# KELVIN-ASU/Lightweight-Multi-Modal-Scene-Understanding-via-Knowledge-Distillation

Measured on AMD Instinct MI355X. Metric: PandaSet 2-class KD training frames/sec, higher is better.
Workload: dtype f32; 1 GPU; KD step: concat-fusion teacher fwd (eval) -> weighted-fusion student fwd/bwd (train BN), CE + T^2*KL(T=4) + feature-MSE, fused AdamW; random-init weights; teacher_fusion=concat, student_fusion=weighted, image=3x256x256, points_per_frame=80000, bev_grid=64x64, num_classes=2, per_gpu_batch=256, global_batch=256, parallelism=dp1

## Files before the change

include/kd_hip.h:

```cpp
#ifndef KD_HIP_H
#define KD_HIP_H
#include <stddef.h>
#include <stdint.h>

#ifdef __cplusplus
extern "C" {
#endif

#define KD_ACT_NONE 0
#define KD_ACT_RELU 1
#define KD_ACT_RELU6 2

int kd_version(void);
const char* kd_arch(void);
const char* kd_last_error_string(void);

int kd_set_gemm_split(int on);
int64_t kd_pwconv_stat_rows(int64_t M);
int64_t kd_pwconv_stat_rows_for(int64_t M, int K, int N, int pro, int epi, int with_addend);
int kd_set_gemm_stream(int mode);
int kd_pwconv_gemm(const float* A, int64_t lda, const float* A2, int64_t lda2, int pro, int pro_act,
                   const float* p0, const float* p1, const float* p2, const float* p3, const float* p4,
                   const float* W, const float* bias, float* C, int64_t ldc, const float* addend,
                   int64_t ldadd, int epi, const float* X, int64_t ldx, const float* esc, const float* esh,
                   const float* emean, const float* einv, int epi_act, float* partial, int64_t partial_rows, int64_t M,
                   int K, int N, const int* m_dev, void* stream);
size_t kd_pwconv_wgrad_ws_bytes(int64_t M, int N, int K);
int kd_set_wgrad_rs(int mode);
int kd_pwconv_wgrad(const float* D, int64_t ldd, const float* X, int64_t ldx, int d_mode, int d_act,
                    const float* al, const float* be, const float* ga, const float* msc, const float* msh,
                    const float* A, int64_t lda, int a_mode, int a_act, const float* asc, const float* ash,
                    float* dW, int64_t M, int N, int K, void* ws, size_t ws_bytes, void* stream);
int kd_transpose(const float* in, float* out, int R, int C, void* stream);
int kd_transpose_batch(const int64_t* table, int n, int nblocks, void* stream);
int kd_copy_segments(const float* s0, float* d0, int64_t n0, const float* s1, float* d1, int64_t n1, const float* s2, float* d2,
                     int64_t n2, const float* s3, float* d3, int64_t n3, void* stream);

int64_t kd_stem_stat_rows(int64_t npix_out);
int kd_stem_conv_fwd(const float* x_nchw, const float* w, float* y_nhwc, float* partial, int B, int Cin, int H,
                     int W, int Cout, void* stream);
int kd_stem_conv_fwd_infer(const float* x_nchw, const float* w, const float* sc, const float* sh, int act, float* y_nhwc,
                           int B, int Cin, int H, int W, int Cout, void* stream);
int kd_stem_im2col(const float* x_nchw, float* col, int B, int Cin, int H, int W, int Kp, void* stream);

int64_t kd_dwconv_stat_rows(int64_t npix_out, int C);
int kd_dwconv3x3_fwd(const float* x, const float* sc, const float* sh, int act, const float* w, float* y,
                     float* partial, int B, int H, int W, int C, int stride, void* stream);
int64_t kd_dwconv_bwd_stat_rows(int64_t npix_in, int C);
int kd_set_dw_bwd_mode(int mode);
size_t kd_dwconv_bwd_ws_bytes(int64_t npix_out, int C);
int kd_dwconv3x3_bwd(const float* D, const float* Y, const float* al, const float* be, const float* ga,
                     const float* dsc, const float* dsh, int d_act, const float* x, const float* sc,
                     const float* sh, int act, const float* mean, const float* invstd, const float* w, float* gx,
                     float* partial, float* dw, int B, int H, int W, int C, int stride, void* ws, size_t ws_bytes,
                     void* stream);
int kd_dwconv3x3_bwd_add_supported(int C, int W, int stride);
int kd_dwconv3x3_bwd_add(const float* D, const float* Y, const float* al, const float* be, const float* ga,
                         const float* dsc, const float* dsh, int d_act, const float* x, const float* sc,
                         const float* sh, int act, const float* mean, const float* invstd, const float* w,
                         const float* addend, float* gx, float* partial, float* dw, int B, int H, int W, int C, int stride,
                         void* ws, size_t ws_bytes, void* stream);

int kd_bn_finalize_train(float* partial, int rows, int C, int pstride, int64_t count, const float* gamma,
                         const float* beta, float eps, float momentum, float* running_mean, float* running_var,
                         int64_t* num_batches_tracked, float* mean, float* invstd, float* scale, float* shift,
                         void* stream);
int kd_bn_eval_coeffs(const float* gamma, const float* beta, const float* running_mean, const float* running_var,
                      float eps, int C, float* mean, float* invstd, float* scale, float* shift, void* stream);
int64_t kd_rowwise_stat_rows(int64_t M, int C);
int kd_bn_act_apply(const float* x, int64_t ldx, const float* sc, const float* sh, int act, const float* res,
                    int64_t ldr, float* out, int64_t ldo, int64_t M, int C, void* stream);
int kd_bn_act_apply_res(const float* x, int64_t ldx, const float* sc, const float* sh, int act, const float* res, int64_t ldr,
                        const float* rsc, const float* rsh, int ract, float* out, int64_t ldo, int64_t M, int C, void* stream);
int kd_bn_bwd_reduce(const float* D, int64_t ldd, const float* X, int64_t ldx, const float* sc, const float* sh,
                     int act, const float* mean, const float* invstd, float* partial, int64_t M, int C,
                     void* stream);
int kd_bn_bwd_finalize(float* partial, int rows, int C, int pstride, int64_t count, const float* gamma, const float* mean,
                       const float* invstd, int training, float* dgamma, float* dbeta, float* al, float* be,
                       float* ga, float* dbias, void* stream);

int kd_lidar_l0_fwd(const float* pts, const float* w, const float* b, float* y, float* partial, int64_t P, int C,
                    const int* p_dev, void* stream);
int kd_lidar_l1_fwd(const float* pts, const float* w0, const float* b0, const float* sc0, const float* sh0, int act0,
                    const float* W1, const float* bias1, float* C, int64_t ldc, int epi, float* partial,
                    int64_t partial_rows, int64_t M, int K, int N, const int* m_dev, void* stream);
// ... 224 lines not shown
```

lightweight-multi-modal-scene-understanding-via-knowledge-distillation_amd/csrc/kd_wgrad_rs.hip:

```cpp
#include "kd_gemm_args.h"

#include <atomic>

int kd_gemm_split_mode();

namespace {

constexpr int RS_THREADS = 512;

__host__ __device__ constexpr int rs_pad(int blk) { return (blk & 1) ? 64 : 32; }
__host__ __device__ constexpr int rs_pitch(int blk) { return 32 * blk + rs_pad(blk); }
__host__ __device__ constexpr int rs_rpp(int cg, int rows) {
  int r = 256 / cg;
  int p = 1;
  while (p * 2 <= r && p * 2 <= rows) p *= 2;
  return p;
}

struct RsGeom {
  int WN, WK;
  int ncs, split_n;
  int nrs;
  int rows_per_slice;
};

template <int TNW, int TKW, int WNc, int WKc, int CHK, int DMODE, int AMODE>
__global__ __launch_bounds__(RS_THREADS, 1) void pw_wgrad_rs_kernel(WgradArgs g, RsGeom q) {
  constexpr int NBLK = TNW * WNc, KBLK = TKW * WKc;
  constexpr int CH = 16 * CHK;
  constexpr int PD = rs_pitch(NBLK), PA = rs_pitch(KBLK);
  constexpr int PLD = CH * PD, PLA = CH * PA;
  constexpr int BUF = 3 * (PLD + PLA);
  constexpr int CGD = 8 * NBLK, CGA = 8 * KBLK;
  constexpr int RPD = rs_rpp(CGD, CH), RPA = rs_rpp(CGA, CH);
  constexpr int ND = CH / RPD, NA = CH / RPA;
  constexpr int NDT = DMODE == 2 ? 2 : 1;
  extern __shared__ __attribute__((aligned(16))) unsigned char smem_raw[];
  unsigned short* lds = reinterpret_cast<unsigned short*>(smem_raw);
  const int tid = threadIdx.x, lane = tid & 63, wave = tid >> 6;
  int cs, rsl;
  {
    const int grp = 8 * q.ncs, g0 = (int)blockIdx.x / grp, r = (int)blockIdx.x % grp;
    if ((g0 + 1) * 8 <= q.nrs) { rsl = g0 * 8 + (r & 7); cs = r >> 3; }
    else { const int rem = q.nrs - g0 * 8; rsl = g0 * 8 + r % rem; cs = r / rem; }
  }
  const int n0 = q.split_n ? cs * 32 * NBLK : 0, k0 = q.split_n ? 0 : cs * 32 * KBLK;
  const int64_t mbeg = (int64_t)rsl * q.rows_per_slice;
  int64_t mend = mbeg + q.rows_per_slice;
  if (mend > g.M) mend = g.M;
  const int nchunk = mbeg < mend ? (int)((mend - mbeg + CH - 1) / CH) : 0;
  const int nstep = (nchunk + 1) & ~1;

  if (wave < 4) {
    constexpr int ACTD = CGD * RPD, ACTA = CGA * RPA;
    static_assert(ACTD >= 128 && ACTA >= 128 && ACTD <= 256 && ACTA <= 256, "lane map");
    const int td = tid < ACTD ? tid : tid - (256 - ACTD), ta = tid < ACTA ? tid : tid - (256 - ACTA);
    const int dcg = td % CGD, drp = td / CGD;
    const int acg = ta % CGA, arp = ta / CGA;
    const int gn = n0 + 4 * dcg, gk = k0 + 4 * acg;
    float4 cd[DMODE == 2 ? 5 : 1], ca[AMODE == 1 ? 2 : 1];
    if (DMODE == 2) {
      cd[0] = kd_ld4(g.al + gn); cd[1] = kd_ld4(g.be + gn); cd[2] = kd_ld4(g.ga + gn);
      cd[3] = kd_ld4(g.msc + gn); cd[4] = kd_ld4(g.msh + gn);
    }
    if (AMODE == 1) { ca[0] = kd_ld4(g.asc + gk); ca[1] = kd_ld4(g.ash + gk); }
    const float* Dp = g.D + n0;
    const float* Xp = DMODE == 2 ? g.X + n0 : nullptr;
    const float* Ap = g.A + k0;
    const int ldd_ = (int)g.ldd, ldx_ = (int)g.ldx, lda_ = (int)g.lda;
    float4 rd[2][NDT][ND], ra[2][NA];
    auto issue = [&](int c, float4 (&sd)[NDT][ND], float4 (&sa)[NA]) __attribute__((always_inline)) {
      const int cc = c < nchunk ? c : (nchunk > 0 ? nchunk - 1 : 0);
      const int64_t m0 = mbeg + (int64_t)cc * CH;
      const int lastrow = (int)(mend - 1 - m0);
      const float* db = Dp + m0 * g.ldd;
      const float* xb = DMODE == 2 ? Xp + m0 * g.ldx : nullptr;
      const float* ab = Ap + m0 * g.lda;
#pragma unroll
      for (int i = 0; i < ND; ++i) {
        const int r = drp + RPD * i, rr = r < lastrow ? r : lastrow;
        sd[0][i] = kd_ld4(db + (unsigned)(rr * ldd_ + 4 * dcg));
        if (DMODE == 2) sd[1][i] = kd_ld4(xb + (unsigned)(rr * ldx_ + 4 * dcg));
      }
#pragma unroll
      for (int i = 0; i < NA; ++i) {
        const int r = arp + RPA * i, rr = r < lastrow ? r : lastrow;
        sa[i] = kd_ld4(ab + (unsigned)(rr * lda_ + 4 * acg));
      }
    };
    auto split_store = [&](float4 v, unsigned short* d, int plane) __attribute__((always_inline)) {
      uint2 hi, mid, lo;
      kd_split3(v, hi, mid, lo);
      *reinterpret_cast<uint2*>(d) = hi;
      *reinterpret_cast<uint2*>(d + plane) = mid;
      *reinterpret_cast<uint2*>(d + 2 * plane) = lo;
    };
    auto convert = [&](int c, const float4 (&sd)[NDT][ND], const float4 (&sa)[NA], int bufi) __attribute__((always_inline)) {
      unsigned short* bd = lds + bufi * BUF;
      unsigned short* ba = bd + 3 * PLD;
      const int64_t m0 = mbeg + (int64_t)c * CH;
      {
#pragma unroll
        for (int i = 0; i < ND; ++i) {
          const int row = drp + RPD * i;
// ... 90 lines not shown
        }
    }
  }
}

std::atomic<int> g_rs_on{1};
int rs_mode() { return g_rs_on.load(std::memory_order_relaxed); }

struct RsPlan { int tnw, tkw, wn, wk, chk, ncs, split_n; };

bool rs_plan(int N, int K, RsPlan& p, bool any = false) {
  if (N % 32 || K % 32) return false;
  int nb = N / 32, kb = K / 32, ncs = 1, split_n = 0;
  if (nb == 24) { nb = 8; ncs = 3; split_n = 1; }
  else if (kb == 24 && nb == 4) { kb = 12; ncs = 2; }
  else if (kb == 24) { kb = 6; ncs = 4; }
  else if (kb == 12 && nb == 4) { }
  else if (kb == 12 && nb <= 4) { kb = 6; ncs = 2; }
  else if (nb == 8 && kb == 8) { nb = 4; ncs = 2; split_n = 1; }
  struct E { int nb, kb, tnw, tkw, wn, wk, chk; };
  static const E tab[] = {
      {6, 1, 3, 1, 2, 1, 2},
      {12, 2, 3, 2, 4, 1, 1},
      {8, 4, 2, 4, 4, 1, 1},
      {2, 6, 1, 3, 2, 2, 2},
      {4, 12, 1, 12, 4, 1, 1},
      {4, 4, 2, 2, 2, 2, 2},
      {4, 2, 2, 1, 2, 2, 2},
      {2, 4, 1, 2, 2, 2, 2},
      {4, 8, 2, 4, 2, 2, 1},
      {2, 8, 1, 4, 2, 2, 2},
  };
  const bool all = any || rs_mode() == 2;
  for (const E& e : tab)
    if (e.nb == nb && e.kb == kb) {
      const bool wins = (nb == 4 && kb == 12) || (nb == 6 && kb == 1) || (nb == 12 && kb == 2) || (nb == 8 && kb == 4) || (nb == 2 && kb == 6 && ncs == 2) ||
                        (nb == 4 && kb == 8);
      if (!wins && !all) return false;
      p = {e.tnw, e.tkw, e.wn, e.wk, e.chk, ncs, split_n};
      return true;
    }
  return false;
}

template <int TNW, int TKW, int WN, int WK, int CHK>
int rs_launch_shape(const WgradArgs& g, const RsGeom& q, hipStream_t st) {
  constexpr int NBLK = TNW * WN, KBLK = TKW * WK;
  constexpr size_t lds = (size_t)2 * 3 * 16 * CHK * (rs_pitch(NBLK) + rs_pitch(KBLK)) * 2;
  static_assert(lds <= 160 * 1024, "the double-buffered plane image must fit the LDS");
  const dim3 grid((unsigned)(q.nrs * q.ncs)), blk(RS_THREADS);
#define KD_RS_CASE(DM_, AM_)                                                                                              \
  if (g.d_mode == DM_ && g.a_mode == AM_) {                                                                               \
    static std::atomic<uint64_t> raised{0};                                                                               \
    const hipError_t e = kd_raise_dynamic_lds((const void*)pw_wgrad_rs_kernel<TNW, TKW, WN, WK, CHK, DM_, AM_>, lds, raised); \
    if (e != hipSuccess) { kd_set_error("kd_wgrad_rs: cannot raise the dynamic LDS limit to %zu B: %s", lds, hipGetErrorString(e)); return -1; } \
    hipLaunchKernelGGL((pw_wgrad_rs_kernel<TNW, TKW, WN, WK, CHK, DM_, AM_>), grid, blk, lds, st, g, q);                  \
    return 1;                                                                                                             \
  }
  KD_RS_CASE(0, 0) KD_RS_CASE(0, 1) KD_RS_CASE(2, 0) KD_RS_CASE(2, 1)
#undef KD_RS_CASE
  return 0;
}

bool rs_enabled() { return rs_mode() != 0; }

int rs_slices(int64_t M, const RsPlan& p) {
  const int ch = 16 * p.chk;
  int nrs = 256 / p.ncs;
  const int64_t chunks = (M + ch - 1) / ch;
  if (nrs > chunks / 8) nrs = (int)(chunks / 8);
  return nrs < 1 ? 1 : nrs;
}

}

extern "C" int kd_set_wgrad_rs(int mode) { return g_rs_on.exchange(mode < 0 ? 0 : (mode > 2 ? 2 : mode)); }

size_t kd_wgrad_rs_ws_bytes(int64_t M, int N, int K) {
  RsPlan p;
  if (!rs_plan(N, K, p, true)) return 0;
  return (size_t)rs_slices(M, p) * (size_t)N * (size_t)K * sizeof(float);
}

int kd_wgrad_rs_launch(const WgradArgs& g0, size_t ws_bytes, float* dW, hipStream_t st) {
  RsPlan p;
  if (!rs_enabled() || !kd_gemm_split_mode() || (g0.d_mode != 0 && g0.d_mode != 2) || g0.a_mode > 1 || !rs_plan(g0.N, g0.K, p)) return 0;
  WgradArgs g = g0;
  const int ch = 16 * p.chk;
  int nrs = rs_slices(g.M, p);
  const size_t cap = ws_bytes / ((size_t)g.N * g.K * sizeof(float));
  if ((size_t)nrs > cap) nrs = (int)cap;
  if (nrs < 1) return 0;
  const int64_t chunks = ((int64_t)g.M + ch - 1) / ch;
  const int64_t cps = (chunks + nrs - 1) / nrs;
  RsGeom q{p.wn, p.wk, p.ncs, p.split_n, 0, (int)(cps * ch)};
  q.nrs = (int)(((int64_t)g.M + q.rows_per_slice - 1) / q.rows_per_slice);
  int rc = 0;
#define KD_RS_SHAPE(A_, B_, C_, D_, E_) if (p.tnw == A_ && p.tkw == B_ && p.wn == C_ && p.wk == D_ && p.chk == E_) rc = rs_launch_shape<A_, B_, C_, D_, E_>(g, q, st);
  KD_RS_SHAPE(3, 1, 2, 1, 2) KD_RS_SHAPE(3, 2, 4, 1, 1) KD_RS_SHAPE(2, 4, 4, 1, 1) KD_RS_SHAPE(1, 3, 2, 2, 2) KD_RS_SHAPE(1, 12, 4, 1, 1)
  KD_RS_SHAPE(2, 2, 2, 2, 2) KD_RS_SHAPE(2, 1, 2, 2, 2) KD_RS_SHAPE(1, 2, 2, 2, 2) KD_RS_SHAPE(2, 4, 2, 2, 1) KD_RS_SHAPE(1, 4, 2, 2, 2)
#undef KD_RS_SHAPE
  if (rc <= 0) return rc;
  const int e = kd_check_launch("kd_wgrad_rs");
  if (e) return -1;
  return kd_slab_reduce_launch(g.slab, q.nrs, (int64_t)g.N * g.K, dW, st) == KD_OK ? 1 : -1;
}
```

lightweight-multi-modal-scene-understanding-via-knowledge-distillation_amd/kdrt/ops.py:

```python
from __future__ import annotations

from typing import Optional, Tuple

import torch

from .lib import KDError, lib, require_gpu_tensor

ACT_NONE, ACT_RELU, ACT_RELU6 = 0, 1, 2
BN_EPS, BN_MOMENTUM = 1e-5, 0.1

_ws = {}
_ws_captured = set()
_ws_keep = []


def stream() -> int:
    return torch.cuda.current_stream().cuda_stream


def workspace(nbytes: int, device) -> torch.Tensor:
    key = (device.type, device.index)
    buf = _ws.get(key)
    capturing = device.type == "cuda" and torch.cuda.is_current_stream_capturing()
    if buf is None or buf.numel() < nbytes:
# ... 207 lines not shown
    t0 = _prof_begin()
    lib.call("kd_lidar_l2_dgrad", P(y), ld(y), P(rows_t), P(grid), P(share), P(al), P(be), P(ga), P(out_op.sc), P(out_op.sh),
             out_op.act, P(Wt), P(gin), ld(gin), P(inp.raw), ld(inp.raw), P(inp.sc), P(inp.sh), P(inp.bnc.mean), P(inp.bnc.invstd),
             inp.act, P(partial), partial_rows, M, N, K, stream())
    _prof_end(t0, "pw_gemm", 2.0 * M * N * K, 4.0 * (M * N + 2 * M * K + M + N * K), None, M)


def l2_bwd(tables, out_op: Operand, Wt, gin, dW, *, inp: Operand, al, be, ga, partial, partial_rows):
    rows_t, grid, share = tables
    y = out_op.raw
    M, N = y.shape
    K = inp.C
    nbytes = lib.kd_lidar_l2_bwd_ws_bytes(M, N, K)
    ws = workspace(nbytes, y.device)
    t0 = _prof_begin()
    lib.call("kd_lidar_l2_bwd", P(y), ld(y), P(rows_t), P(grid), P(share), P(al), P(be), P(ga), P(out_op.sc), P(out_op.sh), out_op.act,
             P(Wt), P(gin), ld(gin), P(inp.raw), ld(inp.raw), P(inp.sc), P(inp.sh), P(inp.bnc.mean), P(inp.bnc.invstd), inp.act,
             P(partial), partial_rows, P(dW), M, N, K, P(ws), nbytes, stream())
    _prof_end(t0, "lidar_bwd", 2.0 * 2.0 * M * N * K, 4.0 * (M * N + 2 * M * K + M + 2 * N * K), None, M)


def l2_wgrad(tables, out_op: Operand, dW, *, inp: Operand, al, be, ga):
    rows_t, grid, share = tables
    y = out_op.raw
    M, N = y.shape
    K = inp.C
    nbytes = lib.kd_pwconv_wgrad_ws_bytes(M, N, K)
    ws = workspace(nbytes, y.device)
    t0 = _prof_begin()
    lib.call("kd_lidar_l2_wgrad", P(y), ld(y), P(rows_t), P(grid), P(share), P(al), P(be), P(ga), P(out_op.sc), P(out_op.sh),
             out_op.act, P(inp.raw), ld(inp.raw), P(inp.sc), P(inp.sh), inp.act, P(dW), M, N, K, P(ws), nbytes, stream())
    _prof_end(t0, "pw_wgrad", 2.0 * M * N * K, 4.0 * (M * N + M * K + M + N * K), None, M)


def l1_wgrad(t, y, dW, *, op: Operand, al, be, ga, msc, msh, mact):
    pts, w0, b0 = op.virt
    M, N, K = pts.shape[0], y.shape[1], w0.shape[0]
    nbytes = lib.kd_pwconv_wgrad_ws_bytes(M, N, K)
    ws = workspace(nbytes, t.device)
    e0 = _prof_begin()
    lib.call("kd_lidar_l1_wgrad", P(t), ld(t), P(y), ld(y), mact, P(al), P(be), P(ga), P(msc), P(msh), P(pts), P(w0), P(b0),
             P(op.sc), P(op.sh), op.act, P(dW), M, N, K, P(ws), nbytes, stream())
    _prof_end(e0, "pw_wgrad", 2.0 * M * N * K, 4.0 * (2 * M * N + M * 4 + N * K), None, M)


def pw_wgrad(D, A, dW, *, M, N, K, X=None, d_mode=0, d_act=0, al=None, be=None, ga=None, msc=None, msh=None,
             a_mode=0, a_act=0, asc=None, ash=None):
    nbytes = lib.kd_pwconv_wgrad_ws_bytes(M, N, K)
    ws = workspace(nbytes, D.device)
    e0 = _prof_begin()
    lib.call("kd_pwconv_wgrad", P(D), ld(D), P(X), ld(X) if X is not None else 0, d_mode, d_act, P(al), P(be), P(ga),
             P(msc), P(msh), P(A), ld(A), a_mode, a_act, P(asc), P(ash), P(dW), M, N, K, P(ws), nbytes, stream())
    _prof_end(e0, "pw_wgrad", 2.0 * M * N * K, 4.0 * (M * N * (2 if d_mode == 2 else 1) + M * K + N * K), None, M)


class TransposeCache:

    def __init__(self):
        self.entries = {}
        self.table = None
        self.nblocks = 0
        self.enabled = True

    @staticmethod
    def _stamp(e):
        o = e[3]()
        return None if o is None else (GLOBAL_EPOCH[0], owner_epoch(o), o._version)

    def get(self, w2d, owner):
        if not self.enabled or owner is None:
            return None
        key = (w2d.data_ptr(), w2d.shape[0], w2d.shape[1])
        e = self.entries.get(key)
        if e is None:
            if torch.cuda.is_current_stream_capturing():
                return None
            R, Cc = w2d.shape
            self.entries[key] = [w2d.detach(), torch.empty(Cc, R, device=w2d.device, dtype=torch.float32), None, _weakref.ref(owner)]
            self.table = None
            return None
        return e[1] if (e[2] is not None and e[2] == self._stamp(e)) else None

    def refresh(self):
        if not self.enabled or not self.entries:
            return
        dead = [k for k, e in self.entries.items() if e[3]() is None]
        if dead and not torch.cuda.is_current_stream_capturing():
            for k in dead:
                del self.entries[k]
            self.table = None
            if not self.entries:
                return
        ents = list(self.entries.values())
        if self.table is None:
            rows, blk = [], 0
            for w, wt, _, _ in ents:
                rows.append([w.data_ptr(), wt.data_ptr(), w.shape[0], w.shape[1], blk])
                blk += (w.numel() + 255) // 256
            if torch.cuda.is_current_stream_capturing():
                return
            self.table = torch.tensor(rows, dtype=torch.int64).to(ents[0][0].device)
            self.nblocks = blk
        lib.call("kd_transpose_batch", P(self.table), len(ents), self.nblocks, stream())
        for e in ents:
            e[2] = self._stamp(e)

# ... 61 lines not shown
```

lightweight-multi-modal-scene-understanding-via-knowledge-distillation_amd/kdrt/units.py:

```python
from __future__ import annotations

import os
from typing import List, Optional, Sequence

import torch

from . import gradsink, ops
from .lib import KDError, lib
from .ops import ACT_NONE, ACT_RELU, BNC, Operand, P, ld, stream


ENCODER_WIDTHS = (8, 16, 24, 32, 40)


def check_encoder_width(base_channels: int) -> None:
    if base_channels not in ENCODER_WIDTHS:
        raise KDError(f"TwinLiteEncoder(base_channels={base_channels}) is not supported: base_channels must be one of "
                      f"{', '.join(map(str, ENCODER_WIDTHS))} (a multiple of 8, at most 40)")


class UnitSpec:

    def __init__(self, kind: str, conv, bn, act: int):
        self.kind, self.conv, self.bn, self.act = kind, conv, bn, act
# ... 244 lines not shown
    n_head = len(units) - 2
    if n_head >= 0:
        head = cur
        for u in units[:n_head]:
            head, _ = unit_forward(u, head, False)
        if dw_pw_tail_ok(units, head):
            return dw_pw_forward_final(units[-2], units[-1], head, res)
        cur = head
        units = units[n_head:]
    for u in units[:-1]:
        cur, _ = unit_forward(u, cur, False)
    return pw_forward_final(units[-1], cur, res), cur.geom


def unit_backward(rec: _Rec, g, need_input_grad: bool = True, addend: Optional[torch.Tensor] = None):
    spec = rec.spec
    y, bnc = rec.y, rec.bnc
    M, C = y.shape if y is not None else (rec.inp.shape[0], rec.w.shape[0])
    out_op = Operand(y, rec.out_geom, bnc, spec.act)
    pstride = None
    if g[0] == "D":
        t = g[1]
        partial, rows = ops.bn_bwd_reduce(t, out_op)
        msc, msh, mact = bnc.scale, bnc.shift, spec.act
        if mact == ACT_NONE:
            msc = msh = None
    else:
        t, partial, rows = g[1], g[2], g[3]
        pstride = g[4] if len(g) > 4 else None
        msc, msh, mact = None, None, ACT_NONE
    tables = g[0] == "GS"
    if tables and not (spec.kind == "pw" and rec.inp.virt is None and rec.inp.bnc is not None):
        raise KDError("table-form scatter gradient needs a pointwise unit with a deferred input")
    beta_p = spec.bn.bias
    g_buf, g_dir = gradsink.out_for(rec.gamma)
    b_buf, b_dir = gradsink.out_for(beta_p)
    want_dbias = spec.has_bias and spec.kind != "l0"
    cb_buf, cb_dir = gradsink.out_for(rec.b) if want_dbias else (None, False)
    dgamma, dbeta, abg, dbias = ops.bn_bwd_finalize(partial, rows, C, M, rec.gamma, bnc, rec.training,
                                                    want_dbias=want_dbias, pstride=pstride, dgamma=g_buf, dbeta=b_buf,
                                                    dbias=cb_buf)
    al, be, ga = abg[0], abg[1], abg[2]
    dev = rec.w.device
    kind = spec.kind
    g_in = None
    if kind == "pw":
        inp = rec.inp
        N, K = C, inp.C
        dW, w_dir = gradsink.out_for(rec.w)
        fused = (tables and need_input_grad and addend is None and lib.kd_lidar_l2_bwd_supported(N, K)
                 and ld(y) == N and ld(inp.raw) == K)
        fused1 = (inp.virt is not None and need_input_grad and addend is None and not tables
                  and mact == ACT_NONE and inp.act == ACT_RELU and lib.kd_lidar_l1_bwd_supported(N, K) and ld(t) == N and ld(y) == N)
        if fused or fused1:
            pass
        elif tables:
            ops.l2_wgrad(t, out_op, dW, inp=inp, al=al, be=be, ga=ga)
        elif inp.virt is not None:
            ops.l1_wgrad(t, y, dW, op=inp, al=al, be=be, ga=ga, msc=msc, msh=msh, mact=mact)
        else:
            ops.pw_wgrad(t, inp.raw, dW, M=M, N=N, K=K, X=y, d_mode=2, d_act=mact, al=al, be=be, ga=ga, msc=msc, msh=msh,
                         a_mode=1 if inp.bnc is not None else 0, a_act=inp.act, asc=inp.sc, ash=inp.sh)
        if need_input_grad:
            Wt = ops.transpose(rec.w.view(N, K), owner=rec.w)
            if fused1:
                rows_in = lib.kd_lidar_l1_bwd_stat_rows(M)
                part_in = torch.empty(rows_in * 2 * K, device=dev, dtype=torch.float32)
                m1 = torch.empty(4, K, device=dev, dtype=torch.float32)
                ops.l1_bwd(t, y, Wt, dW, op=inp, al=al, be=be, ga=ga, partial=part_in, partial_rows=rows_in, moments=m1)
                g_in = ("GM", m1, part_in, rows_in)
            elif inp.virt is not None:
                if addend is not None:
                    raise KDError("addend on a virtual LiDAR layer-0 input is not supported")
                rows_in = lib.kd_lidar_l1_dgrad_stat_rows(M, N, K)
                part_in = torch.empty(rows_in * 2 * K, device=dev, dtype=torch.float32)
                m1 = torch.empty(4, K, device=dev, dtype=torch.float32)
                ops.l1_dgrad(t, y, Wt, None, op=inp, al=al, be=be, ga=ga, msc=msc, msh=msh, mact=mact, partial=part_in,
                             partial_rows=rows_in, moments=m1)
                g_in = ("GM", m1, part_in, rows_in)
            elif fused:
                gin = torch.empty(M, K, device=dev, dtype=torch.float32)
                rows_in = lib.kd_lidar_l2_bwd_stat_rows(M)
                part_in = torch.empty(rows_in * 2 * K, device=dev, dtype=torch.float32)
                ops.l2_bwd(t, out_op, Wt, gin, dW, inp=inp, al=al, be=be, ga=ga, partial=part_in, partial_rows=rows_in)
                g_in = ("G", gin, part_in, rows_in)
            elif tables:
                gin = torch.empty(M, K, device=dev, dtype=torch.float32)
                rows_in = lib.kd_lidar_l2_dgrad_stat_rows(M, N, K)
                part_in = torch.empty(rows_in * 2 * K, device=dev, dtype=torch.float32)
                ops.l2_dgrad(t, out_op, Wt, gin, inp=inp, al=al, be=be, ga=ga, partial=part_in, partial_rows=rows_in)
                g_in = ("G", gin, part_in, rows_in)
            elif inp.bnc is not None:
                gin = torch.empty(M, K, device=dev, dtype=torch.float32)
                rows_in = lib.kd_pwconv_stat_rows_for(M, N, K, 2, 2, int(addend is not None))
                part_in = torch.empty(rows_in * 2 * K, device=dev, dtype=torch.float32)
                ops.pw_gemm(t, Wt, gin, M=M, K=N, N=K, A2=y, pro=2, pro_act=mact, p=(al, be, ga, msc, msh),
                            addend=addend, epi=2, X=inp.raw, esc=inp.sc, esh=inp.sh, emean=inp.bnc.mean,
                            einv=inp.bnc.invstd, epi_act=inp.act, partial=part_in, partial_rows=rows_in)
                g_in = ("G", gin, part_in, rows_in)
            else:
                dx = torch.empty(M, K, device=dev, dtype=torch.float32)
                ops.pw_gemm(t, Wt, dx, M=M, K=N, N=K, A2=y, pro=2, pro_act=mact, p=(al, be, ga, msc, msh),
                            addend=addend, epi=0)
                g_in = dx
        grads = [gradsink.finish(rec.w, dW, w_dir)]
    elif kind == "dw":
        inp = rec.inp
        B, H, W = inp.geom
        s = spec.stride
        npix_out = M
        dW, w_dir = gradsink.out_for(rec.w)
        nbytes = lib.kd_dwconv_bwd_ws_bytes(npix_out, C)
        ws = ops.workspace(nbytes, dev)
        gx = part_in = None
        rows_in = 0
        deferred = inp.bnc is not None
        if need_input_grad:
            gx = torch.empty(inp.M, C, device=dev, dtype=torch.float32)
# ... 517 lines not shown
    return SameHeadFn.apply(x, list(units), training, cls_conv.weight, cls_conv.bias, *_params_of(units))


class X4HeadFn(torch.autograd.Function):

    @staticmethod
    def forward(ctx, x, units, training, wc, bc, *params):
        xm, geom = ops.nhwc_view(x)
        cur = Operand(xm, geom)
        recs = []
        for u in units:
            cur, rec = unit_forward(u, cur, training)
            recs.append(rec)
        B, H, W = cur.geom
        NC, Cin = wc.shape[0], wc.shape[1]
        logits = torch.empty(B, NC, H, W, device=xm.device, dtype=torch.float32)
        lib.call("kd_cls3x3_fwd", P(cur.raw), P(cur.sc), P(cur.sh), cur.act, P(wc), P(bc), P(logits), B, H, W, Cin, NC,
                 stream())
        ctx.recs, ctx.last, ctx.wc, ctx.bc = recs, cur, wc, bc
        return logits

    @staticmethod
    def backward(ctx, dlog):
        dlog = dlog.contiguous()
        cur, wc = ctx.last, ctx.wc
        B, H, W = cur.geom
        NC, Cin = wc.shape[0], wc.shape[1]
        M = cur.M
        dev = dlog.device
        gx = torch.empty(M, Cin, device=dev, dtype=torch.float32)
        rows = lib.kd_cls3x3_bwd_stat_rows(M, Cin)
        partial = torch.empty(rows * 2 * Cin, device=dev, dtype=torch.float32)
        nw = NC * Cin * 9
        dwb = torch.empty(nw + 4, device=dev, dtype=torch.float32)
        nbytes = lib.kd_cls3x3_bwd_ws_bytes(M, Cin, NC)
        ws = ops.workspace(nbytes, dev)
        lib.call("kd_cls3x3_bwd", P(dlog), P(cur.raw), P(cur.sc), P(cur.sh), cur.act, P(cur.bnc.mean), P(cur.bnc.invstd),
                 P(wc), P(gx), P(partial), P(dwb), B, H, W, Cin, NC, P(ws), nbytes, stream())
        grads, g_in = chain_backward(ctx.recs, ("G", gx, partial, rows), need_input_grad=ctx.needs_input_grad[0])
        dx = ops.nchw_from_matrix(g_in, ctx.recs[0].inp.geom) if ctx.needs_input_grad[0] else None
        dwc, dbc = gradsink.deliver_many([(wc, dwb[:nw]), (ctx.bc, dwb[nw: nw + NC])])
        return (dx, None, None, dwc, dbc,
                *grads)


def run_x4_head(x, units, cls_conv, training):
    return X4HeadFn.apply(x, list(units), training, cls_conv.weight, cls_conv.bias, *_params_of(units))


_SCATTER_MODE = "sorted"
_SCATTER_TABLES = True
_SCATTER_HOLDERS = True
_LIDAR_FUSED_INFER = True


_sort_cache: dict = {}
_sort_sharing = False


def share_point_bins(on: bool):
    global _sort_sharing
    _sort_sharing = bool(on)
    _sort_cache.clear()


def clear_step_caches():
    _sort_cache.clear()


def cell_sort(pts, B, N, H, W, rng):
    key = (pts.data_ptr(), pts._version, B, N, H, W, tuple(float(r) for r in rng), stream())
    hit = _sort_cache.get("entry") if _sort_sharing else None
    if hit is not None and hit[0] == key:
        return hit[2]
    dev = pts.device
    row_of_point = torch.empty(B * N, device=dev, dtype=torch.int32)
    seg_start = torch.empty(B * H * W + 1, device=dev, dtype=torch.int32)
    perm = torch.empty(B * N, device=dev, dtype=torch.int32)
    nbytes = lib.kd_lidar_cell_sort_ws_bytes(B, N, H, W)
    ws = ops.workspace(nbytes, dev)
    lib.call("kd_lidar_cell_sort", P(pts), B, N, H, W, float(rng[0]), float(rng[1]), float(rng[2]), float(rng[3]),
             P(row_of_point), P(seg_start), P(perm), P(ws), nbytes, stream())
    out = (row_of_point, seg_start, perm)
    if _sort_sharing:
        _sort_cache["entry"] = (key, pts, out)
    return out


SORT_MAX_BINS = 36865
SORT_WIDE_MAX_DIM = 4096
_SORT_WIDE = os.environ.get("KD_LIDAR_WIDE_SORT", "1") != "0"


def sorted_mode_available(H, W):
    return H * W + 1 <= SORT_MAX_BINS or (_SORT_WIDE and max(H, W) <= SORT_WIDE_MAX_DIM)


def sort_points(pts, B, N, H, W, rng):
    fn = "kd_lidar_sort_points" if H * W + 1 <= SORT_MAX_BINS else "kd_lidar_sort_points_wide"
    key = ("points", pts.data_ptr(), pts._version, B, N, H, W, tuple(float(r) for r in rng), stream())
    hit = _sort_cache.get("points") if _sort_sharing else None
    if hit is not None and hit[0] == key:
        return hit[2]
    dev = pts.device
    spts = torch.empty(B * N, 4, device=dev, dtype=torch.float32)
    row_sorted = torch.empty(B * N, device=dev, dtype=torch.int32)
# ... 139 lines not shown
```

Measured before the change: 3601 frames/s.

## Fuse pointwise-conv data gradient into the row-sliced weight-gradient kernel

Adds a data-gradient role to the row-sliced weight-gradient kernel for the 192x32 pointwise shape. An extra wave reuses the already-staged split-bf16 D tiles in LDS and multiplies them by the transposed weights held in registers, writing dX directly. This removes a separate GEMM launch and a second read of the output gradient for eligible layers (no BN-input transform, no addend, no tables). It is limited to one shape, and the extra wave may lengthen each block's critical path.

```diff
diff --git a/include/kd_hip.h b/include/kd_hip.h
--- a/include/kd_hip.h
+++ b/include/kd_hip.h
@@ -31,6 +31,13 @@
                     const float* al, const float* be, const float* ga, const float* msc, const float* msh,
                     const float* A, int64_t lda, int a_mode, int a_act, const float* asc, const float* ash,
                     float* dW, int64_t M, int N, int K, void* ws, size_t ws_bytes, void* stream);
+int kd_pwconv_bwd_supported(int N, int K, int d_mode, int a_mode, int epi);
+size_t kd_pwconv_bwd_ws_bytes(int64_t M, int N, int K);
+int kd_pwconv_bwd(const float* D, int64_t ldd, const float* X, int64_t ldx, int d_mode, int d_act,
+                  const float* al, const float* be, const float* ga, const float* msc, const float* msh,
+                  const float* A, int64_t lda, int a_mode, int a_act, const float* asc, const float* ash,
+                  const float* Wt, float* dX, int64_t lddx, const float* addend, int64_t ldadd, int epi,
+                  float* dW, int64_t M, int N, int K, void* ws, size_t ws_bytes, void* stream);
 int kd_transpose(const float* in, float* out, int R, int C, void* stream);
 int kd_transpose_batch(const int64_t* table, int n, int nblocks, void* stream);
 int kd_copy_segments(const float* s0, float* d0, int64_t n0, const float* s1, float* d1, int64_t n1, const float* s2, float* d2,
diff --git a/lightweight-multi-modal-scene-understanding-via-knowledge-distillation_amd/csrc/kd_wgrad_rs.hip b/lightweight-multi-modal-scene-understanding-via-knowledge-distillation_amd/csrc/kd_wgrad_rs.hip
--- a/lightweight-multi-modal-scene-understanding-via-knowledge-distillation_amd/csrc/kd_wgrad_rs.hip
+++ b/lightweight-multi-modal-scene-understanding-via-knowledge-distillation_amd/csrc/kd_wgrad_rs.hip
@@ -24,8 +24,14 @@
   int rows_per_slice;
 };
 
-template <int TNW, int TKW, int WNc, int WKc, int CHK, int DMODE, int AMODE>
-__global__ __launch_bounds__(RS_THREADS, 1) void pw_wgrad_rs_kernel(WgradArgs g, RsGeom q) {
+struct RsDgrad {
+  const float* Wt;
+  float* dX;
+  float* dump;
+};
+
+template <int TNW, int TKW, int WNc, int WKc, int CHK, int DMODE, int AMODE, int DG>
+__global__ __launch_bounds__(RS_THREADS, 1) void pw_wgrad_rs_kernel(WgradArgs g, RsGeom q, RsDgrad dg) {
   constexpr int NBLK = TNW * WNc, KBLK = TKW * WKc;
   constexpr int CH = 16 * CHK;
   constexpr int PD = rs_pitch(NBLK), PA = rs_pitch(KBLK);
@@ -50,6 +56,57 @@
   if (mend > g.M) mend = g.M;
   const int nchunk = mbeg < mend ? (int)((mend - mbeg + CH - 1) / CH) : 0;
   const int nstep = (nchunk + 1) & ~1;
+
+  if constexpr (DG != 0) {
+    static_assert(TNW == 3 && TKW == 1 && WNc == 2 && WKc == 1 && CHK == 2 && AMODE == 0, "the data-gradient role exists for the 192 x 32 plan only");
+    if (wave == 6) {
+      constexpr int KSN = 2 * NBLK;
+      constexpr int PAo[6] = {0, 2, 1, 0, 1, 0}, PBo[6] = {2, 0, 1, 1, 0, 0};
+      const int r = lane & 31, h = lane >> 5;
+      bf16x8 wp[KSN][3];
+      {
+        const float* wrow = dg.Wt + r * (32 * NBLK) + 8 * h;
+#pragma unroll
+        for (int ks = 0; ks < KSN; ++ks) {
+          uint2 h0, m0_, l0, h1, m1_, l1;
+          kd_split3(kd_ld4(wrow + 16 * ks), h0, m0_, l0);
+          kd_split3(kd_ld4(wrow + 16 * ks + 4), h1, m1_, l1);
+          wp[ks][0] = __builtin_bit_cast(bf16x8, make_uint4(h0.x, h0.y, h1.x, h1.y));
+          wp[ks][1] = __builtin_bit_cast(bf16x8, make_uint4(m0_.x, m0_.y, m1_.x, m1_.y));
+          wp[ks][2] = __builtin_bit_cast(bf16x8, make_uint4(l0.x, l0.y, l1.x, l1.y));
+        }
+      }
+      const int foff = r * PD + 8 * h;
+      const int ooff = 4 * h * (32 * KBLK) + r;
+      float* const dlane = dg.dump + lane;
+      kd_lds_barrier();
+      for (int s = 0; s < nstep; ++s) {
+        const unsigned short* bd = lds + (s & 1) * BUF + foff;
+        f32x16 acc;
+#pragma unroll
+        for (int i = 0; i < 16; ++i) acc[i] = 0.f;
+#pragma unroll
+        for (int ks = 0; ks < KSN; ++ks) {
+          bf16x8 a[3];
+#pragma unroll
+          for (int p = 0; p < 3; ++p) a[p] = *reinterpret_cast<const bf16x8*>(bd + p * PLD + 16 * ks);
+#pragma unroll
+          for (int t = 0; t < 6; ++t) acc = __builtin_amdgcn_mfma_f32_32x32x16_bf16(a[PAo[t]], wp[ks][PBo[t]], acc, 0, 0, 0);
+        }
+        kd_lds_barrier();
+        const int64_t m0 = mbeg + (int64_t)s * CH;
+        const int left = s < nchunk ? (int)(mend - m0) : 0;
+        float* const ob = dg.dX + m0 * (32 * KBLK) + ooff;
+#pragma unroll
+        for (int i = 0; i < 16; ++i) {
+          const int row = (i & 3) + 8 * (i >> 2);
+          float* const dst = row + 4 * h < left ? ob + row * (32 * KBLK) : dlane;
+          if (DG == 2) __builtin_nontemporal_store(acc[i], dst); else *dst = acc[i];
+        }
+      }
+      return;
+    }
+  }
 
   if (wave < 4) {
     constexpr int ACTD = CGD * RPD, ACTA = CGA * RPA;
@@ -246,9 +303,9 @@
 #define KD_RS_CASE(DM_, AM_)                                                                                              \
   if (g.d_mode == DM_ && g.a_mode == AM_) {                                                                               \
     static std::atomic<uint64_t> raised{0};                                                                               \
-    const hipError_t e = kd_raise_dynamic_lds((const void*)pw_wgrad_rs_kernel<TNW, TKW, WN, WK, CHK, DM_, AM_>, lds, raised); \
+    const hipError_t e = kd_raise_dynamic_lds((const void*)pw_wgrad_rs_kernel<TNW, TKW, WN, WK, CHK, DM_, AM_, 0>, lds, raised); \
     if (e != hipSuccess) { kd_set_error("kd_wgrad_rs: cannot raise the dynamic LDS limit to %zu B: %s", lds, hipGetErrorString(e)); return -1; } \
-    hipLaunchKernelGGL((pw_wgrad_rs_kernel<TNW, TKW, WN, WK, CHK, DM_, AM_>), grid, blk, lds, st, g, q);                  \
+    hipLaunchKernelGGL((pw_wgrad_rs_kernel<TNW, TKW, WN, WK, CHK, DM_, AM_, 0>), grid, blk, lds, st, g, q, RsDgrad{});    \
     return 1;                                                                                                             \
   }
   KD_RS_CASE(0, 0) KD_RS_CASE(0, 1) KD_RS_CASE(2, 0) KD_RS_CASE(2, 1)
@@ -266,6 +323,19 @@
   return nrs < 1 ? 1 : nrs;
 }
 
+RsGeom rs_geom(int64_t M, const RsPlan& p, int nrs0) {
+  const int ch = 16 * p.chk;
+  const int64_t chunks = (M + ch - 1) / ch;
+  const int64_t cps = (chunks + nrs0 - 1) / nrs0;
+  RsGeom q{p.wn, p.wk, p.ncs, p.split_n, 0, (int)(cps * ch)};
+  q.nrs = (int)((M + q.rows_per_slice - 1) / q.rows_per_slice);
+  return q;
+}
+
+constexpr int BWD_N = 192, BWD_K = 32, BWD_DUMP = 64;
+
+bool bwd_plan(RsPlan& p) { return rs_plan(BWD_N, BWD_K, p) && p.tnw == 3 && p.tkw == 1 && p.wn == 2 && p.wk == 1 && p.chk == 2 && p.ncs == 1; }
+
 }
 
 extern "C" int kd_set_wgrad_rs(int mode) { return g_rs_on.exchange(mode < 0 ? 0 : (mode > 2 ? 2 : mode)); }
@@ -280,15 +350,11 @@
   RsPlan p;
   if (!rs_enabled() || !kd_gemm_split_mode() || (g0.d_mode != 0 && g0.d_mode != 2) || g0.a_mode > 1 || !rs_plan(g0.N, g0.K, p)) return 0;
   WgradArgs g = g0;
-  const int ch = 16 * p.chk;
   int nrs = rs_slices(g.M, p);
   const size_t cap = ws_bytes / ((size_t)g.N * g.K * sizeof(float));
   if ((size_t)nrs > cap) nrs = (int)cap;
   if (nrs < 1) return 0;
-  const int64_t chunks = ((int64_t)g.M + ch - 1) / ch;
-  const int64_t cps = (chunks + nrs - 1) / nrs;
-  RsGeom q{p.wn, p.wk, p.ncs, p.split_n, 0, (int)(cps * ch)};
-  q.nrs = (int)(((int64_t)g.M + q.rows_per_slice - 1) / q.rows_per_slice);
+  const RsGeom q = rs_geom(g.M, p, nrs);
   int rc = 0;
 #define KD_RS_SHAPE(A_, B_, C_, D_, E_) if (p.tnw == A_ && p.tkw == B_ && p.wn == C_ && p.wk == D_ && p.chk == E_) rc = rs_launch_shape<A_, B_, C_, D_, E_>(g, q, st);
   KD_RS_SHAPE(3, 1, 2, 1, 2) KD_RS_SHAPE(3, 2, 4, 1, 1) KD_RS_SHAPE(2, 4, 4, 1, 1) KD_RS_SHAPE(1, 3, 2, 2, 2) KD_RS_SHAPE(1, 12, 4, 1, 1)
@@ -299,3 +365,68 @@
   if (e) return -1;
   return kd_slab_reduce_launch(g.slab, q.nrs, (int64_t)g.N * g.K, dW, st) == KD_OK ? 1 : -1;
 }
+
+
+extern "C" {
+
+int kd_pwconv_bwd_supported(int N, int K, int d_mode, int a_mode, int epi) {
+  RsPlan p;
+  return N == BWD_N && K == BWD_K && (d_mode == 0 || d_mode == 2) && a_mode == 0 && epi == 0 && kd_gemm_split_mode() && rs_enabled() && bwd_plan(p);
+}
+
+size_t kd_pwconv_bwd_ws_bytes(int64_t M, int N, int K) {
+  RsPlan p;
+  if (N != BWD_N || K != BWD_K || M < 1 || !bwd_plan(p)) return 0;
+  return ((size_t)rs_slices(M, p) * (size_t)N * (size_t)K + BWD_DUMP) * sizeof(float);
+}
+
+int kd_pwconv_bwd(const float* D, int64_t ldd, const float* X, int64_t ldx, int d_mode, int d_act, const float* al,
+                  const float* be, const float* ga, const float* msc, const float* msh, const float* A, int64_t lda,
+                  int a_mode, int a_act, const float* asc, const float* ash, const float* Wt, float* dX, int64_t lddx,
+                  const float* addend, int64_t ldadd, int epi, float* dW, int64_t M, int N, int K, void* ws, size_t ws_bytes,
+                  void* stream) {
+  KD_REQUIRE(D && A && Wt && dX && dW && ws && M > 0 && N > 0 && K > 0, KD_ERR_ARG, "kd_pwconv_bwd: null pointer or empty shape");
+  KD_REQUIRE(kd_pwconv_bwd_supported(N, K, d_mode, a_mode, epi), KD_ERR_SHAPE,
+             "kd_pwconv_bwd: no instance for N=%d K=%d d_mode=%d a_mode=%d epi=%d in the %s arithmetic%s (use kd_pwconv_wgrad + kd_pwconv_gemm)",
+             N, K, d_mode, a_mode, epi, kd_gemm_split_mode() ? "split" : "exact-fp32", rs_enabled() ? "" : " with kd_set_wgrad_rs(0)");
+  KD_REQUIRE(!addend, KD_ERR_ARG, "kd_pwconv_bwd: no instance with an addend (ldadd=%lld) (use kd_pwconv_wgrad + kd_pwconv_gemm)", (long long)ldadd);
+  KD_REQUIRE(M < (int64_t)1 << 31, KD_ERR_SHAPE, "kd_pwconv_bwd: M too large");
+  KD_REQUIRE(ldd == N && (d_mode != 2 || ldx == N) && lda == K && lddx == K, KD_ERR_SHAPE,
+             "kd_pwconv_bwd: D, X, A and dX must be dense matrices (row strides %lld, %lld, %lld, %lld)", (long long)ldd, (long long)ldx,
+             (long long)lda, (long long)lddx);
+  if (d_mode == 2) KD_REQUIRE(X && al && be && ga, KD_ERR_ARG, "kd_pwconv_bwd: d_mode 2 needs X, al, be, ga");
+  if (d_mode == 2 && d_act != KD_ACT_NONE) KD_REQUIRE(msc && msh, KD_ERR_ARG, "kd_pwconv_bwd: mask needs sc/sh");
+  KD_REQUIRE(kd_aligned16(D) && kd_aligned16(X) && kd_aligned16(A) && kd_aligned16(Wt) && kd_aligned16(dX) && kd_aligned16(ws) &&
+             kd_aligned16(al) && kd_aligned16(be) && kd_aligned16(ga) && kd_aligned16(msc) && kd_aligned16(msh), KD_ERR_ALIGN,
+             "kd_pwconv_bwd: 16-byte alignment");
+  KD_REQUIRE(ws_bytes >= kd_pwconv_bwd_ws_bytes(M, N, K), KD_ERR_WORKSPACE, "kd_pwconv_bwd: workspace too small (%zu B)", ws_bytes);
+  if (d_mode == 2 && !msc) { msc = al; msh = al; }
+  RsPlan p;
+  bwd_plan(p);
+  const int nrs0 = rs_slices(M, p);
+  const RsGeom q = rs_geom(M, p, nrs0);
+  float* slab = (float*)ws;
+  WgradArgs g{D, ldd, X, ldx, al, be, ga, msc, msh, d_mode, d_act, A, lda, asc, ash, a_mode, a_act, slab, (int)M, N, K, 0, nullptr, nullptr};
+  const RsDgrad dgr{Wt, dX, slab + (size_t)nrs0 * N * K};
+  const int nt = kd_nt_store((size_t)M * K * sizeof(float));
+  constexpr size_t lds = (size_t)2 * 3 * 32 * (rs_pitch(6) + rs_pitch(1)) * 2;
+  const dim3 grid((unsigned)q.nrs), blk(RS_THREADS);
+  hipStream_t st = (hipStream_t)stream;
+  bool launched = false;
+#define KD_BWD_CASE(DM_, DG_)                                                                                             \
+  if (d_mode == DM_ && nt + 1 == DG_) {                                                                                   \
+    static std::atomic<uint64_t> raised{0};                                                                               \
+    const hipError_t e = kd_raise_dynamic_lds((const void*)pw_wgrad_rs_kernel<3, 1, 2, 1, 2, DM_, 0, DG_>, lds, raised);  \
+    KD_REQUIRE(e == hipSuccess, (int)e, "kd_pwconv_bwd: cannot raise the dynamic LDS limit to %zu B: %s", lds, hipGetErrorString(e)); \
+    hipLaunchKernelGGL((pw_wgrad_rs_kernel<3, 1, 2, 1, 2, DM_, 0, DG_>), grid, blk, lds, st, g, q, dgr);                  \
+    launched = true;                                                                                                      \
+  }
+  KD_BWD_CASE(0, 1) KD_BWD_CASE(0, 2) KD_BWD_CASE(2, 1) KD_BWD_CASE(2, 2)
+#undef KD_BWD_CASE
+  KD_REQUIRE(launched, KD_ERR_ARG, "kd_pwconv_bwd: no kernel for d_mode=%d", d_mode);
+  const int rc = kd_check_launch("kd_pwconv_bwd");
+  if (rc) return rc;
+  return kd_slab_reduce_launch(slab, q.nrs, (int64_t)N * K, dW, st);
+}
+
+}
diff --git a/lightweight-multi-modal-scene-understanding-via-knowledge-distillation_amd/kdrt/ops.py b/lightweight-multi-modal-scene-understanding-via-knowledge-distillation_amd/kdrt/ops.py
--- a/lightweight-multi-modal-scene-understanding-via-knowledge-distillation_amd/kdrt/ops.py
+++ b/lightweight-multi-modal-scene-understanding-via-knowledge-distillation_amd/kdrt/ops.py
@@ -283,6 +283,18 @@
     lib.call("kd_pwconv_wgrad", P(D), ld(D), P(X), ld(X) if X is not None else 0, d_mode, d_act, P(al), P(be), P(ga),
              P(msc), P(msh), P(A), ld(A), a_mode, a_act, P(asc), P(ash), P(dW), M, N, K, P(ws), nbytes, stream())
     _prof_end(e0, "pw_wgrad", 2.0 * M * N * K, 4.0 * (M * N * (2 if d_mode == 2 else 1) + M * K + N * K), None, M)
+
+
+def pw_bwd(D, A, Wt, dX, dW, *, M, N, K, X=None, d_mode=0, d_act=0, al=None, be=None, ga=None, msc=None, msh=None,
+           a_mode=0, a_act=0, asc=None, ash=None, addend=None, epi=0):
+    nbytes = lib.kd_pwconv_bwd_ws_bytes(M, N, K)
+    ws = workspace(nbytes, D.device)
+    e0 = _prof_begin()
+    lib.call("kd_pwconv_bwd", P(D), ld(D), P(X), ld(X) if X is not None else 0, d_mode, d_act, P(al), P(be), P(ga),
+             P(msc), P(msh), P(A), ld(A), a_mode, a_act, P(asc), P(ash), P(Wt), P(dX), ld(dX), P(addend),
+             ld(addend) if addend is not None else 0, epi, P(dW), M, N, K, P(ws), nbytes, stream())
+    _prof_end(e0, "pw_bwd", 4.0 * M * N * K,
+              4.0 * (M * N * (2 if d_mode == 2 else 1) + 2 * M * K + (addend is not None) * M * K + 2 * N * K), None, M)
 
 
 class TransposeCache:
diff --git a/lightweight-multi-modal-scene-understanding-via-knowledge-distillation_amd/kdrt/units.py b/lightweight-multi-modal-scene-understanding-via-knowledge-distillation_amd/kdrt/units.py
--- a/lightweight-multi-modal-scene-understanding-via-knowledge-distillation_amd/kdrt/units.py
+++ b/lightweight-multi-modal-scene-understanding-via-knowledge-distillation_amd/kdrt/units.py
@@ -320,7 +320,10 @@
                  and ld(y) == N and ld(inp.raw) == K)
         fused1 = (inp.virt is not None and need_input_grad and addend is None and not tables
                   and mact == ACT_NONE and inp.act == ACT_RELU and lib.kd_lidar_l1_bwd_supported(N, K) and ld(t) == N and ld(y) == N)
-        if fused or fused1:
+        a_mode = 1 if inp.bnc is not None else 0
+        fused_pw = (_PW_BWD_FUSED and need_input_grad and not tables and inp.virt is None and inp.bnc is None and addend is None
+                    and lib.kd_pwconv_bwd_supported(N, K, 2, a_mode, 0) and ld(t) == N and ld(y) == N and ld(inp.raw) == K)
+        if fused or fused1 or fused_pw:
             pass
         elif tables:
             ops.l2_wgrad(t, out_op, dW, inp=inp, al=al, be=be, ga=ga)
@@ -328,10 +331,15 @@
             ops.l1_wgrad(t, y, dW, op=inp, al=al, be=be, ga=ga, msc=msc, msh=msh, mact=mact)
         else:
             ops.pw_wgrad(t, inp.raw, dW, M=M, N=N, K=K, X=y, d_mode=2, d_act=mact, al=al, be=be, ga=ga, msc=msc, msh=msh,
-                         a_mode=1 if inp.bnc is not None else 0, a_act=inp.act, asc=inp.sc, ash=inp.sh)
+                         a_mode=a_mode, a_act=inp.act, asc=inp.sc, ash=inp.sh)
         if need_input_grad:
             Wt = ops.transpose(rec.w.view(N, K), owner=rec.w)
-            if fused1:
+            if fused_pw:
+                dx = torch.empty(M, K, device=dev, dtype=torch.float32)
+                ops.pw_bwd(t, inp.raw, Wt, dx, dW, M=M, N=N, K=K, X=y, d_mode=2, d_act=mact, al=al, be=be, ga=ga, msc=msc, msh=msh,
+                           a_mode=0, a_act=inp.act)
+                g_in = dx
+            elif fused1:
                 rows_in = lib.kd_lidar_l1_bwd_stat_rows(M)
                 part_in = torch.empty(rows_in * 2 * K, device=dev, dtype=torch.float32)
                 m1 = torch.empty(4, K, device=dev, dtype=torch.float32)
@@ -955,6 +963,7 @@
 _SCATTER_TABLES = True
 _SCATTER_HOLDERS = True
 _LIDAR_FUSED_INFER = True
+_PW_BWD_FUSED = True
 
 
 _sort_cache: dict = {}
```

Measured after the change: 3642 frames/s, median of 6. 1.1% higher.
